# Starfish-develop/Starfish

Hardware: AMD Instinct MI355X
Metric: log-likelihood evals/sec, 4096-pixel order, batch=128 walkers (higher is better)
Workload: dtype f64; 1 GPU; cfg2: synthetic single order N_pix=4096, 8 eigenspectra, M=27, N_f=8192, 1 global + 1 local kernel, all 13 parameters thawed, batch=128 walkers per GPU; global_batch=128, units_per_gpu=128, parallelism=(order x walker) units sharded x1, one process per GPU, no data-path collective

## Files before the change

starfish_amd/csrc/sf_chol_dataflow.h:

```cpp
#pragma once
#include "sf_chol_host.h"
#include "sf_chol_diag.h"
#include "sf_chol_sync.h"
#include "sf_chol_panel.h"

struct sf_df_stage {
    int off;
    int St;
    int Sr;
    int thr_pt;
    int thr_rp;
    int dep;
    int fw;
};
struct sf_df_stage_packed {
    int off;
    unsigned short thr_pt, thr_rp, fw;
    unsigned char split;
    signed char dep;
};
static_assert(sizeof(sf_df_stage_packed) == 12, "sf_df_stage_packed");
template <class S>
__host__ __device__ __forceinline__ sf_df_stage sf_df_stage_of(S& x) {
    sf_df_stage r;
    r.off = x.off;
    const int sp = x.split;
    r.St = sp & 15;
    r.Sr = sp >> 4;
    r.thr_pt = x.thr_pt;
    r.thr_rp = x.thr_rp;
    r.dep = x.dep;
    r.fw = x.fw;
    return r;
}
static inline sf_df_stage_packed sf_df_pack(const sf_df_stage& x) {
    sf_df_stage_packed r;
    r.off = x.off;
    r.thr_pt = (unsigned short)x.thr_pt;
    r.thr_rp = (unsigned short)x.thr_rp;
    r.fw = (unsigned short)x.fw;
    r.split = (unsigned char)(x.St | (x.Sr << 4));
    r.dep = (signed char)x.dep;
    return r;
}
#define SF_DF_QUEUES 8
#define SF_DF_MAX_STAGES 127
#define SF_DF_FRONT_MAX 6
#define SF_DF_FRONT_WIDEST 3
#define SF_DF_QTILES (2 * SF_CHIP_WGS / SF_DF_QUEUES)
struct sf_df_args {
    sf_panel_args p;
    int nt, batch, front;
    int fstart[SF_DF_FRONT_MAX];
    int thr_base[2][2][SF_DF_FRONT_MAX];
    int fp_pos;
    int bq[2], ntasks[2];
    int pt_cap;
    int *head, *abort_flag, *done_top, *done_D, *done_row, *row_L, *fp_cnt, *rp_cnt, *stage_done;
    int* chain_next;
    double* T;
    int64_t sT;
    double* part;
    int* info;
    int qbal;
    long long* diag;
    long long* dbg;
    int miss_claims;
    long long* trace;
    long long trace_cap;
    sf_df_stage_packed st[2][SF_DF_MAX_STAGES];
};
static_assert(sizeof(sf_df_args) <= 4096, "kernel arguments of k_potrf_dataflow");
#define SF_DF_LDS_DOUBLES ((37 * DBS + 128) > (4 * GT * GLD + 2 * GT) ? (37 * DBS + 128) : (4 * GT * GLD + 2 * GT))
#define SF_DF_LDS_BYTES ((SF_DF_LDS_DOUBLES + 4) * sizeof(double))

typedef const __attribute__((address_space(4))) sf_df_args sf_df_kargs;
#define SF_DF_HELPER __attribute__((noinline))
#define SF_DF_PROGRESS() sf_df_add(a.abort_flag + 5, 1)
#ifdef SF_TUNING
#define SF_DF_MISS_CLAIMS(x) ((a.miss_claims & 1) && (x))
#else
#define SF_DF_MISS_CLAIMS(x) (false)
#endif
__device__ SF_DF_HELPER bool sf_df_try_chain(sf_df_kargs& a, const int qx, int& cb, int& ck, int& cd) {
    const int nt = a.nt, F = a.front;
    const int Bq = (a.batch - qx + SF_DF_QUEUES - 1) / SF_DF_QUEUES;
    const int vq = Bq == a.bq[0] ? 0 : 1;
    for (int dd = 1; dd <= F; ++dd) {
        for (int j = 0; j < Bq; ++j) {
            const int b1 = qx + SF_DF_QUEUES * j;
            int* ctr = a.chain_next + SF_DF_FRONT_MAX * b1 + dd - 1;
            const int k1 = sf_df_load(ctr);
            const int kp = dd == 1 ? k1 - 1 : k1 + a.fstart[dd - 1];
            if (dd == 1 ? k1 >= nt : kp + dd > nt - 1) continue;
            bool ready = true;
            if (kp >= 0) {
                ready = sf_df_load(a.done_top + b1) >= kp;
                if (ready && kp >= 1) {
                    ready = sf_df_load(a.row_L + (size_t)b1 * nt + kp + dd) >= kp;
                    const int St = a.st[vq][kp - 1].split & 15;
                    if (ready && St > 0)
                        ready = sf_df_load(a.fp_cnt + 2 * SF_DF_FRONT_MAX * b1 + SF_DF_FRONT_MAX * (kp & 1) + dd - 1) >=
                                a.st[vq][kp - 1].thr_pt - a.thr_base[vq][kp & 1][dd - 1];
                }
            }
            if (!ready) continue;
            int expect = k1;
            if (__hip_atomic_compare_exchange_strong(ctr, &expect, k1 + 1, __ATOMIC_RELAXED, __ATOMIC_RELAXED,
                                                     __HIP_MEMORY_SCOPE_AGENT)) {
                cb = b1;
                ck = dd == 1 ? k1 : kp;
                cd = dd;
                return true;
            }
        }
    }
    return false;
}

template <bool RHS>
__global__ __launch_bounds__(512, 4) void k_potrf_dataflow(const sf_df_args a_in) {
    extern __shared__ __attribute__((aligned(16))) double dsm[];
    double* sm = dsm;
    double(*red)[GT] = (double(*)[GT])(dsm + 4 * GT * GLD);
    int* s_ints = (int*)(dsm + SF_DF_LDS_DOUBLES);
    const size_t region = sf_split_region_tiles_dev() * (size_t)(GT * GT);
    sf_df_kargs* ap = (sf_df_kargs*)__builtin_amdgcn_kernarg_segment_ptr();
    (void)a_in;
    int qcur = (int)(blockIdx.x & (SF_DF_QUEUES - 1));
    {
        const int nb = ap->batch, big = nb % SF_DF_QUEUES;
        if (ap->qbal && big != 0) {
            if (nb < SF_DF_QUEUES && SF_DF_QUEUES % nb == 0) {
                qcur = qcur % nb;
            } else {
                const int mine = (nb - qcur + SF_DF_QUEUES - 1) / SF_DF_QUEUES;
                const int slot = (int)(blockIdx.x >> 3);
                const int keep = (int)(((long long)mine * gridDim.x + nb / 2) / nb);
                if (qcur >= big && slot >= keep) qcur = (slot - keep + qcur) % big;
            }
        }
    }
    int visited = 0;
    int kst = 0;
    if (threadIdx.x == 0) {
        s_ints[5] = 0;
        s_ints[6] = 0;
        sf_df_add(ap->abort_flag + 6, 1);
        if (blockIdx.x == 0)
            __hip_atomic_store((long long*)(ap->abort_flag + 8), (long long)ap->diag, __ATOMIC_RELAXED, __HIP_MEMORY_SCOPE_AGENT);
    }
    int pend_t = -1, resume = 0;
    for (;;) {
        int tid = threadIdx.x;
        asm volatile("" : "+v"(tid));
        sf_df_kargs& a = *ap;
        const int nt = a.nt, F = a.front;
        const int n = a.p.n, fp = a.p.fp;
        const int B = (a.batch - qcur + SF_DF_QUEUES - 1) / SF_DF_QUEUES;
        const int v = B == a.bq[0] ? 0 : 1;
        const int ntasks = B > 0 ? a.ntasks[v] : 0;
        if (resume) {
            resume = 0;
        } else if (pend_t >= 0) {
            if (tid == 0) s_ints[0] = pend_t;
            pend_t = -1;
        } else if (tid == 0) {
            int t = -1, cb = 0, ck = 0, cd = 1;
            if (sf_df_load(a.abort_flag) == 0) {
                t = -2;
                auto try_chain = [&](int qx) { return SF_DF_MISS_CLAIMS(visited < SF_DF_QUEUES) ? false : sf_df_try_chain(a, qx, cb, ck, cd); };
                if (try_chain(qcur)) {
                    t = -3;
                } else if (visited < SF_DF_QUEUES) {
                    t = ntasks > 0 ? __hip_atomic_fetch_add(a.head + qcur, 1, __ATOMIC_RELAXED, __HIP_MEMORY_SCOPE_AGENT) : ntasks;
                    if (t >= ntasks) t = -4;
                } else {
                    bool live = false;
                    for (int qx = 0; qx < SF_DF_QUEUES && t == -2; ++qx)
                        if (try_chain(qx)) {
                            t = -3;
                            s_ints[5] = 0;
                        }
                    if (t == -2) {
                        for (int b1 = 0; b1 < a.batch; ++b1) {
                            live = live || sf_df_load(a.chain_next + SF_DF_FRONT_MAX * b1) < nt;
                            for (int dd = 2; dd <= F; ++dd)
                                live = live || sf_df_load(a.chain_next + SF_DF_FRONT_MAX * b1 + dd - 1) + a.fstart[dd - 1] + dd <= nt - 1;
                        }
                        if (!live) {
                            t = -5;
                        } else {
                            const int now = (int)((wall_clock64() >> 20) & 0x3fffffff) + 1;
                            const int pg = sf_df_load(a.abort_flag + 5);
                            if (s_ints[5] == 0 || pg != s_ints[6]) {
                                s_ints[5] = now;
                                s_ints[6] = pg;
                            }
                            const int idle = (now - s_ints[5]) & 0x3fffffff;
                            const int stall = (int)(sf_df_stall_ticks(a.abort_flag) >> 20);
                            if (idle > stall) {
                                sf_df_report(a.abort_flag, a.chain_next, nt, SF_DF_ABORT_STALL, (long long)idle << 20);
                                t = -1;
                            }
                            __builtin_amdgcn_s_sleep(64);
                        }
                    }
                }
            }
            s_ints[0] = t;
            s_ints[2] = cb;
            s_ints[3] = ck;
            s_ints[4] = cd;
        }
        __syncthreads();
        const int t = __builtin_amdgcn_readfirstlane(s_ints[0]);
        const int chain_b = __builtin_amdgcn_readfirstlane(s_ints[2]), chain_k = __builtin_amdgcn_readfirstlane(s_ints[3]);
        const int chain_d = __builtin_amdgcn_readfirstlane(s_ints[4]);
        __syncthreads();
        if (t == -1) {
            if (a.info)
                for (int bb = tid; bb < a.batch; bb += 512) a.info[bb] = SF_INFO_INTERNAL;
            return;
        }
        if (t == -5) return;
        if (t == -2) continue;
// ... 617 lines not shown
```

starfish_amd/csrc/sf_chol_host.h:

```cpp
#pragma once
#include "sf_chol_tile.h"

#define SF_TSKEW 40
#define SF_CHIP_WGS 512
#define SF_SPLIT_MAX 8
static size_t sf_split_region_tiles(void) { return 2 * SF_CHIP_WGS; }
__device__ __forceinline__ size_t sf_split_region_tiles_dev(void) { return 2 * SF_CHIP_WGS; }
static int sf_split_policy(long long wgs, int nk) {
    int S = 1;
    while (2 * S <= SF_SPLIT_MAX && wgs * 2 * S <= 384 && nk / (2 * S) >= 8) S *= 2;
    return S;
}
struct sf_potrf_scratch {
    double* T;
    int64_t sT;
    double* W;
    int64_t sW;
    double* part;
    int batch;
    size_t doubles;
    double* Wbuf(int i) const { return W + (size_t)i * batch * sW; }
    size_t Wdoubles() const { return 2 * (size_t)batch * sW; }
    double* Wslot(int k) const { return Wbuf((k >> 1) & 1) + (size_t)(k & 1) * GT * SF_LDT; }
};
static sf_potrf_scratch sf_potrf_scratch_of(double* work, int n, int batch) {
    sf_potrf_scratch w = {};
    const size_t b = (size_t)batch;
    w.sT = (int64_t)(n + SF_NB) * SF_LDT + SF_TSKEW;
    w.sW = (int64_t)SF_NB * SF_LDT + SF_TSKEW;
    w.batch = batch;
    const size_t oT = b * SF_LTB_DOUBLES, oW = oT + b * w.sT, opart = oW + w.Wdoubles() + 64;
    w.doubles = opart + (size_t)(SF_EXEC_GROUPS + 1) * sf_split_region_tiles() * (GT * GT);
    if (work) {
        w.T = work + oT;
        w.W = work + oW;
        w.part = work + opart;
    }
    return w;
}
size_t sf_potrf_work_doubles(int n, int batch) { return sf_potrf_scratch_of(nullptr, n, batch).doubles; }

template <class Args>
static void sf_set_gen(Args& g, const sf_gen_args* gen, int fp) {
    if (!gen) return;
    g.genY = gen->Y - fp;
    g.sY = (int64_t)gen->mpad * gen->ldy;
    g.ldy = gen->ldy;
    g.mpad = gen->mpad;
    g.tilemap = gen->tilemap;
    g.nt128 = gen->nt128;
}
template <class Args>
static Args sf_panel_frame(double* A, int n, int lda, int64_t stride, double* rhs, int ldr, const sf_gen_args* gen, int fp) {
    Args g = {};
    g.C = A;
    g.sC = stride;
    g.lda = lda;
    g.n = n;
    g.rhs = rhs;
    g.ldr = ldr;
    g.fp = fp;
    sf_set_gen(g, gen, fp);
    return g;
}

#define SF_TRY(x)          \
    do {                   \
        int rc__ = (x);    \
        if (rc__) return rc__; \
    } while (0)
static int sf_exec_fork(sf_exec* ex, hipStream_t s, std::initializer_list<hipStream_t> to) {
    hipEvent_t e;
    SF_TRY(sf_exec_event(ex, &e));
    SF_HIP(hipEventRecord(e, s));
    for (hipStream_t t : to) SF_HIP(hipStreamWaitEvent(t, e, 0));
    return SF_OK;
}
static int sf_exec_join(sf_exec* ex, hipStream_t s, hipStream_t c, std::initializer_list<hipEvent_t> also = {}) {
    hipEvent_t e;
    SF_TRY(sf_exec_event(ex, &e));
    SF_HIP(hipEventRecord(e, c));
    SF_HIP(hipStreamWaitEvent(s, e, 0));
    for (hipEvent_t x : also)
        if (x) SF_HIP(hipStreamWaitEvent(s, x, 0));
    return SF_OK;
}
```

starfish_amd/csrc/sf_chol_panel.h:

```cpp
#pragma once
#include "sf_device.h"
#include "sf_chol_tile.h"

struct sf_panel_args {
    double* C;
    int64_t sC;
    int lda, n;
    int k0, pw;
    int row0, nslab;
    int slab_step;
    int ksplit, kchunk;
    double* part;
    const double* Wt;
    int64_t sW;
    double* rhs;
    int ldr;
    double* Sout;
    int64_t sS;
    int ldS;
    const double* genY;
    const unsigned char* tilemap;
    int64_t sY;
    int ldy, mpad, nt128;
    int kband, nband, xrow0;
    int fp;
    int prio;
    int kstop, ktail;
    const int* wflag;
    int wval;
    int* abort_flag;
};

struct sf_panel_task {
    int k0, pw, row0, nslab, slab_step;
    int ksplit, kchunk, kstop, ktail;
    double* part;
    const double* Wt;
    int64_t sW;
    double* Sout;
    const int* wflag;
    int wval;
    int* abort_flag;
    int* lds_int;
    int* top_flag;
    int top_val;
    const int* sflag;
    int sval;
    long long* stamps;
    int prio;
};
__device__ __forceinline__ sf_panel_task sf_task_of(const sf_panel_args& g) {
    sf_panel_task q;
    q.k0 = g.k0;
    q.pw = g.pw;
    q.row0 = g.row0;
    q.nslab = g.nslab;
    q.slab_step = g.slab_step;
    q.ksplit = g.ksplit;
    q.kchunk = g.kchunk;
    q.kstop = g.kstop;
    q.ktail = g.ktail;
    q.part = g.part;
    q.Wt = g.Wt;
    q.sW = g.sW;
    q.Sout = g.Sout;
    q.wflag = g.wflag;
    q.wval = g.wval;
    q.abort_flag = g.abort_flag;
    q.lds_int = nullptr;
    q.top_flag = nullptr;
    q.top_val = 0;
    q.sflag = nullptr;
    q.sval = 0;
    q.stamps = nullptr;
    q.prio = g.prio;
    return q;
}

__device__ __forceinline__ const double* sf_uniform_ptr(const double* p) {
    const unsigned long long v = (unsigned long long)p;
    const unsigned lo = __builtin_amdgcn_readfirstlane((unsigned)v), hi = __builtin_amdgcn_readfirstlane((unsigned)(v >> 32));
    return (const double*)(((unsigned long long)hi << 32) | lo);
}

__device__ __forceinline__ int sf_swz(int row) {
    const int t = (row >> 1) & 7;
    return t ^ ((((t >> 1) ^ (t >> 2)) & 1) << 1);
}

template <int NI_LO>
__device__ __forceinline__ void sf_solve_step(sf_d4 (&acc)[2][4], const double* Ab, const double* Bb) {
#pragma unroll
    for (int ks = 0; ks < 4; ++ks) {
        double a[2], bb[4];
#pragma unroll
        for (int i = 0; i < 2; ++i) a[i] = Ab[i * 16 * CLD + ks * 4];
#pragma unroll
        for (int i = NI_LO; i < 4; ++i) bb[i] = Bb[i * 16 * GLD + ks * 4];
#pragma unroll
        for (int mi = 0; mi < 2; ++mi)
#pragma unroll
            for (int ni = NI_LO; ni < 4; ++ni)
                acc[mi][ni] = __builtin_amdgcn_mfma_f64_16x16x4f64(a[mi], bb[ni], acc[mi][ni], 0, 0, 0);
    }
}

template <bool RHS, int MODE, class GA>
__device__ __forceinline__ void sf_panel_body(GA& g, const sf_panel_task& tk, const int id, double* __restrict__ sm,
                                              double (*red)[GT], const int tid) {
    constexpr int TM = 2, TN = 4;
    double(*As)[GT * GLD] = (double(*)[GT * GLD]) sm;
    double(*Bs)[GT * GLD] = (double(*)[GT * GLD])(sm + 2 * GT * GLD);
    double* Ach = sm;

    const int tile = __builtin_amdgcn_readfirstlane(MODE == 1 ? id / tk.ksplit : id);
    const int sp = __builtin_amdgcn_readfirstlane(MODE == 1 ? id - tile * tk.ksplit : 0);
    const int b = __builtin_amdgcn_readfirstlane(tile / tk.nslab);
    const int sl = tile - b * tk.nslab;
    const int row0 = (g.xrow0 && sl == tk.nslab - 1) ? g.xrow0 : tk.row0 + sl * tk.slab_step * GT;
    const int rows_here = min(GT, ((g.nband && row0 < g.nband) ? g.nband : g.n) - row0);
    const int pw = tk.pw, k0 = tk.k0;
    const int cfp = k0 == 0 ? g.fp : 0;
    if (tk.prio) __builtin_amdgcn_s_setprio(2);

    const int lane = tid & 63;
    const int w = __builtin_amdgcn_readfirstlane(tid >> 6);
    const int wm = w >> 1, wn = (w ^ (w >> 2)) & 1;
    const int l15 = lane & 15, lq = lane >> 4;
    double* Cb = g.C + (int64_t)b * g.sC;

    sf_d4 acc[TM][TN];
    if (pw > 0) {
        const int lr = tid >> 3, lc = (tid & 7) * 2;
        const double* Ap[2];
        const double* Bp[2];
#pragma unroll
        for (int p = 0; p < 2; ++p) {
            Ap[p] = Cb + (int64_t)(row0 + min(lr + 64 * p, rows_here - 1)) * g.lda + lc;
            Bp[p] = Cb + (int64_t)(k0 + min(lr + 64 * p, pw - 1)) * g.lda + lc;
        }
        const int grow = lane >> 3, gpos = lane & 7;
        unsigned Aoff[2], Boff[2];
        const double* Abase = sf_uniform_ptr(Cb + (int64_t)row0 * g.lda);
        const double* Bbase = sf_uniform_ptr(Cb + (int64_t)k0 * g.lda);
#pragma unroll
        for (int q = 0; q < 2; ++q) {
            const int row = 16 * w + 8 * q + grow;
            const int c = gpos ^ sf_swz(row);
            Aoff[q] = (unsigned)(min(row, rows_here - 1) * g.lda + 2 * c) * 8u;
            Boff[q] = (unsigned)(min(row, pw - 1) * g.lda + 2 * c) * 8u;
        }
        typedef __attribute__((address_space(3))) void* lds_ptr;
        double* A2 = sm;
        double* B2 = sm + 2 * GT * GK;
        const unsigned ldsA = (unsigned)(size_t)(lds_ptr)A2, ldsB = (unsigned)(size_t)(lds_ptr)B2;
// ... 231 lines not shown
#ifdef SF_TUNING
                if (tk.stamps) tk.stamps[2] = wall_clock64();
#endif
            }
        }
        if (RHS && g.rhs) {
            const double* z = g.rhs + (int64_t)b * g.ldr + k0;
            double zc[TN];
#pragma unroll
            for (int ni = 0; ni < TN; ++ni) {
                const int col = wn * (16 * TN) + ni * 16 + l15;
                zc[ni] = (col < pw && col >= cfp) ? z[col] : 0.0;
            }
#pragma unroll
            for (int mi = 0; mi < TM; ++mi)
#pragma unroll
                for (int r = 0; r < 4; ++r) {
                    double v = 0.0;
#pragma unroll
                    for (int ni = 0; ni < TN; ++ni) v = __builtin_fma(acc[mi][ni][r], zc[ni], v);
                    v += __shfl_xor(v, 1);
                    v += __shfl_xor(v, 2);
                    v += __shfl_xor(v, 4);
                    v += __shfl_xor(v, 8);
                    if (l15 == 0) red[wn][wm * (16 * TM) + mi * 16 + lq + 4 * r] = v;
                }
        }
    }

    {
        const int p = w >> 1, h = w & 1;
        int bi[5], bj[5];
#pragma unroll
        for (int q = 0; q < 5; ++q) {
            if (h == 0) {
                bi[q] = 7 - p;
                bj[q] = q;
            } else {
                const int n_hi = 3 - p;
                const int qq = q < 4 ? q : 0;
                bi[q] = qq < n_hi ? 7 - p : p;
                bj[q] = qq < n_hi ? 5 + qq : qq - n_hi;
            }
        }
        const int nstore = h == 0 ? 5 : 4;
        const int nk2 = pw / GK;
        const int lr = tid >> 3, lc = (tid & 7) * 2;
        const double* Lp[2];
#pragma unroll
        for (int q = 0; q < 2; ++q) Lp[q] = Cb + (int64_t)(row0 + min(lr + 64 * q, rows_here - 1)) * g.lda + k0 + lc;
        double2 rl[2];
        auto gload2 = [&](int kt) {
#pragma unroll
            for (int q = 0; q < 2; ++q) rl[q] = kt * GK + lc >= cfp ? *(const double2*)(Lp[q] + kt * GK) : make_double2(0.0, 0.0);
        };
        auto lstore2 = [&](int buf) {
#pragma unroll
            for (int q = 0; q < 2; ++q) {
                double* pa = &As[buf][(lr + 64 * q) * GLD + lc];
                pa[0] = rl[q].x;
                pa[1] = rl[q].y;
            }
        };
        if (tk.sflag && !sf_df_wait(tk.sflag, tk.sval, tk.abort_flag, tid, tk.lds_int)) return;
#ifdef SF_TUNING
        if (tk.stamps && tid == 0) tk.stamps[3] = wall_clock64();
#endif
        __syncthreads();
        if (nk2 > 0) gload2(0);
        const double* Sin = Cb + (int64_t)row0 * g.lda + row0;
        sf_d4 acc2[5];
        const bool full_tile = rows_here == GT && row0 >= g.fp;
        if (full_tile) {
#pragma unroll
            for (int q = 0; q < 5; ++q)
#pragma unroll
                for (int r = 0; r < 4; ++r) {
                    const int row = 16 * bi[q] + lq + 4 * r, col = 16 * bj[q] + l15;
                    acc2[q][r] = Sin[(int64_t)row * g.lda + col];
                }
        } else {
#pragma unroll
            for (int q = 0; q < 5; ++q)
#pragma unroll
                for (int r = 0; r < 4; ++r) {
                    const int row = 16 * bi[q] + lq + 4 * r, col = 16 * bj[q] + l15;
                    if (row0 + min(row, col) < g.fp)
                        acc2[q][r] = row == col ? 1.0 : 0.0;
                    else
                        acc2[q][r] = (q < nstore && row < rows_here && col < rows_here) ? Sin[(int64_t)row * g.lda + col] : 0.0;
                }
        }
        if (nk2 > 0) lstore2(0);
        __syncthreads();
        auto compute2 = [&](int cur) {
            const double* S = &As[cur][l15 * GLD + lq];
#pragma unroll
            for (int ks = 0; ks < GK / 4; ++ks) {
#pragma unroll
                for (int q = 0; q < 5; ++q)
                    acc2[q] = __builtin_amdgcn_mfma_f64_16x16x4f64(S[bi[q] * 16 * GLD + ks * 4], S[bj[q] * 16 * GLD + ks * 4],
                                                                   acc2[q], 0, 0, 1);
            }
        };
        for (int kt = 0; kt + 1 < nk2; ++kt) {
            gload2(kt + 1);
            compute2(kt & 1);
            lstore2((kt & 1) ^ 1);
            __syncthreads();
        }
        if (nk2 > 0) compute2((nk2 - 1) & 1);
        const bool parked = tk.Sout && sl == 0;
        double* So = parked ? tk.Sout + (int64_t)b * g.sS : Cb + (int64_t)row0 * g.lda + row0;
        const int ldo = parked ? g.ldS : g.lda;
        if (full_tile) {
#pragma unroll
            for (int q = 0; q < 4; ++q)
#pragma unroll
                for (int r = 0; r < 4; ++r) {
                    const int row = 16 * bi[q] + lq + 4 * r, col = 16 * bj[q] + l15;
                    So[(int64_t)row * ldo + col] = acc2[q][r];
                }
            if (nstore == 5) {
#pragma unroll
                for (int r = 0; r < 4; ++r) {
                    const int row = 16 * bi[4] + lq + 4 * r, col = 16 * bj[4] + l15;
                    So[(int64_t)row * ldo + col] = acc2[4][r];
                }
            }
        } else {
#pragma unroll
            for (int q = 0; q < 5; ++q) {
                if (q >= nstore) continue;
#pragma unroll
                for (int r = 0; r < 4; ++r) {
                    const int row = 16 * bi[q] + lq + 4 * r, col = 16 * bj[q] + l15;
                    if (row < rows_here && col < rows_here) So[(int64_t)row * ldo + col] = acc2[q][r];
                }
            }
        }
    }
    if (RHS && g.rhs && pw > 0) {
        __syncthreads();
        if (tid < rows_here) g.rhs[(int64_t)b * g.ldr + row0 + tid] -= red[0][tid] + red[1][tid];
    }
}

template <bool RHS, int MODE>
__global__ __launch_bounds__(512, 4) void k_chol_panel(sf_panel_args g) {
    __shared__ __attribute__((aligned(16))) double sm[4 * GT * GLD];
    __shared__ double red[2][GT];
    sf_panel_body<RHS, MODE>(g, sf_task_of(g), sf_xcd_remap(blockIdx.x, gridDim.x), sm, red, threadIdx.x);
}
```

starfish_amd/csrc/sf_chol_seq.h:

```cpp
#pragma once
#include "sf_chol_host.h"
#include "sf_chol_diag.h"
#include "sf_chol_panel.h"
#include "sf_chol_wide.h"

static int sf_check_front_pad(int fp, int n) {
    if (fp != 0 && (fp != 64 || n % GT != 64)) {
        sf_set_error("potrf: front pad %d does not fit n = %d", fp, n);
        return SF_EINVAL;
    }
    return SF_OK;
}

template <class Args>
static void sf_park(Args& g, const sf_potrf_scratch& ws) {
    g.Sout = ws.T;
    g.sS = ws.sT;
    g.ldS = SF_LDT;
}
static double sf_slab_rows(int n, int row0, int nslab, int step) {
    double rows = 0.0;
    for (int i = 0; i < nslab; ++i) {
        const int r0 = row0 + i * step * GT;
        rows += (n - r0 < GT) ? n - r0 : GT;
    }
    return rows;
}
static int sf_check_grid(long long nblk) {
    if (nblk > 0x7fffffffLL) {
        sf_set_error("panel grid too large");
        return SF_EINVAL;
    }
    return SF_OK;
}

static int sf_panel_split(int k0, int pw, int fp, long long nblk) {
    return pw > 0 ? sf_split_policy(nblk, (k0 > fp ? k0 - fp : 0) / GK) : 1;
}
static int sf_panel_step(sf_panel_args g, const sf_potrf_scratch& ws, int k0, int pw, int row0, int nslab, int step, const double* Wt,
                         bool to_scratch, hipStream_t st, int region, int phase) {
    const int n = g.n, fp = g.fp, batch = ws.batch;
    g.k0 = k0;
    g.pw = pw;
    g.row0 = row0;
    g.nslab = nslab;
    g.slab_step = step;
    g.Wt = Wt;
    g.sW = ws.sW;
    if (to_scratch) {
        sf_park(g, ws);
        g.prio = 1;
    }
    const long long nblk = (long long)nslab * batch;
    SF_TRY(sf_check_grid(nblk));
    const double rows = sf_slab_rows(n, row0, nslab, step);
    const double flops_main = 2.0 * (k0 > fp ? k0 - fp : 0) * rows * pw * batch;
    const double flops_epi = (rows * pw * (double)pw + (double)GT * rows * pw) * batch;
    const int nk = (k0 > fp ? k0 - fp : 0) / GK;
    const int S = sf_panel_split(k0, pw, fp, nblk);
    void* tok;
    if (S > 1) {
        g.ksplit = S;
        g.kchunk = (nk + S - 1) / S;
        g.part = ws.part + (size_t)region * sf_split_region_tiles() * (GT * GT);
        if (phase != 2) {
            sf_prof_gemm_begin(st, flops_main, &tok);
            hipLaunchKernelGGL((k_chol_panel<false, 1>), dim3((unsigned)(nblk * S)), dim3(512), 0, st, g);
            sf_prof_gemm_end(tok);
        }
        if (phase != 1) {
            sf_prof_gemm_begin(st, flops_epi, &tok);
            if (g.rhs)
                hipLaunchKernelGGL((k_chol_panel<true, 2>), dim3((unsigned)nblk), dim3(512), 0, st, g);
            else
                hipLaunchKernelGGL((k_chol_panel<false, 2>), dim3((unsigned)nblk), dim3(512), 0, st, g);
            sf_prof_gemm_end(tok);
        }
    } else {
        sf_prof_gemm_begin(st, flops_main + flops_epi, &tok);
        if (g.rhs)
            hipLaunchKernelGGL((k_chol_panel<true, 0>), dim3((unsigned)nblk), dim3(512), 0, st, g);
        else
            hipLaunchKernelGGL((k_chol_panel<false, 0>), dim3((unsigned)nblk), dim3(512), 0, st, g);
        sf_prof_gemm_end(tok);
    }
    SF_LAUNCH_CHECK();
    return SF_OK;
}

struct sf_wide_stamps {
#ifdef SF_TUNING
    long long* t = nullptr;
    int n = 0, k[64];
#endif
};
#ifdef SF_TUNING
static int sf_wide_stamps_begin(sf_wide_stamps& w) {
    if (SF_TUNE_FLAG("SF_WIDE_STAMPS")) {
        SF_HIP(hipHostMalloc((void**)&w.t, sizeof(long long) * 16 * 64));
        for (int i = 0; i < 16 * 64; ++i) w.t[i] = 0;
    }
    return SF_OK;
}
static void sf_wide_stamps_report(sf_wide_stamps& w, hipStream_t s) {
    if (!w.t) return;
    (void)hipStreamSynchronize(s);
    fprintf(stderr, "wide launches, workgroup grid/2: k nslab | prologue | K loop | solve 1 | 2b | solve 2 | store + rhs | S load + step 4 | S store + drain | total (us)\n");
    for (int i = 0; i < w.n; ++i) {
        const long long* t = w.t + 16 * i;
        fprintf(stderr, "%2d %2d |", w.k[i] / 1000, w.k[i] % 1000);
        const int seg[8][2] = {{0, 1}, {1, 2}, {2, 3}, {3, 4}, {4, 5}, {5, 6}, {6, 7}, {7, 8}};
        for (auto& sg : seg) fprintf(stderr, " %7.1f |", (t[sg[1]] - t[sg[0]]) / 100.0);
        fprintf(stderr, " %7.1f\n", (t[8] - t[0]) / 100.0);
    }
    (void)hipHostFree(w.t);
}
#else
static int sf_wide_stamps_begin(sf_wide_stamps&) { return SF_OK; }
static void sf_wide_stamps_report(sf_wide_stamps&, hipStream_t) {}
#endif

static int sf_panel_step_w(sf_panelw_args g, const sf_potrf_scratch& ws, int k, int slab0, int nslab, int step, bool park, hipStream_t st,
                           sf_wide_stamps& stamps) {
    const int n = g.n, fp = g.fp, batch = ws.batch;
    g.k0 = k * GT;
    g.row0 = slab0 * GT;
    g.nslab = nslab;
    g.slab_step = step;
    g.Wt0 = ws.Wslot(k);
    g.Wt1 = ws.Wslot(k + 1);
    g.sW = ws.sW;
    if (park) sf_park(g, ws);
    const long long nblk = (long long)nslab * batch;
    SF_TRY(sf_check_grid(nblk));
#ifdef SF_TUNING
    if (stamps.t && stamps.n < 64) {
        stamps.k[stamps.n] = k * 1000 + nslab;
        g.stamps = stamps.t + 16 * stamps.n++;
    }
#endif
    const double rows = sf_slab_rows(n, g.row0, nslab, step);
    const double kk = g.k0 > fp ? g.k0 - fp : 0;
    const double flops = (2.0 * kk * rows * GT + 2.0 * (kk + GT) * rows * GT + 2.0 * (rows * GT * (double)GT + (double)GT * rows * GT)) * batch;
    void* tok;
    sf_prof_gemm_begin(st, flops, &tok);
    if (g.rhs)
        hipLaunchKernelGGL(k_chol_panel_w<true>, dim3((unsigned)nblk), dim3(1024), SF_PANELW_LDS, st, g);
    else
        hipLaunchKernelGGL(k_chol_panel_w<false>, dim3((unsigned)nblk), dim3(1024), SF_PANELW_LDS, st, g);
    sf_prof_gemm_end(tok);
    SF_LAUNCH_CHECK();
    return SF_OK;
}

static int sf_diag_step(const sf_potrf_scratch& ws, double* A, int lda, int64_t stride, double* rhs, int ldr, int* info, int n, int k,
                        double* Wt, int fp, hipStream_t st) {
    const int k0 = k * GT;
    const int pw = (n - k0 < GT) ? n - k0 : GT;
    return sf_launch_diag128(ws.T, ws.sT, pw, info, k0 - fp, rhs ? rhs + k0 : nullptr, ldr, A + (int64_t)k0 * lda + k0, lda, stride, Wt,
                             ws.sW, ws.batch, st, k == 0 ? fp : 0);
}

struct sf_narrow_events {
    hipEvent_t d, rest[2];
};
static int sf_narrow_step(const sf_panel_args& base, const sf_potrf_scratch& ws, sf_exec* ex, int* info, int k, double* Wt, hipStream_t c,
                          const hipStream_t gs[2], const hipEvent_t last[2], hipEvent_t* e_top, sf_narrow_events* ev) {
    const int n = base.n, fp = base.fp, nt = (n + GT - 1) / GT;
    const int k0 = k * GT;
    const int pw = (n - k0 < GT) ? n - k0 : GT;
    *ev = {};
    SF_TRY(sf_diag_step(ws, base.C, base.lda, base.sC, base.rhs, base.ldr, info, n, k, Wt, fp, c));
    if (k + 1 >= nt) return SF_OK;
    SF_TRY(sf_exec_event(ex, &ev->d));
    SF_HIP(hipEventRecord(ev->d, c));
    const int gk = (k + 1) & 1;
    if (e_top && sf_panel_split(k0, pw, fp, ws.batch) > 1) {
        if (*e_top) SF_HIP(hipStreamWaitEvent(gs[gk], *e_top, 0));
        SF_TRY(sf_panel_step(base, ws, k0, pw, (k + 1) * GT, 1, 1, Wt, true, gs[gk], 0, 1));
        hipEvent_t e_part;
        SF_TRY(sf_exec_event(ex, &e_part));
        SF_HIP(hipEventRecord(e_part, gs[gk]));
        SF_HIP(hipStreamWaitEvent(c, e_part, 0));
        SF_TRY(sf_panel_step(base, ws, k0, pw, (k + 1) * GT, 1, 1, Wt, true, c, 0, 2));
    } else {
        if (last[gk]) SF_HIP(hipStreamWaitEvent(c, last[gk], 0));
        SF_TRY(sf_panel_step(base, ws, k0, pw, (k + 1) * GT, 1, 1, Wt, true, c, 0, 0));
    }
    if (e_top) {
        SF_TRY(sf_exec_event(ex, e_top));
        SF_HIP(hipEventRecord(*e_top, c));
    }
    for (int g = 0; g < 2; ++g) {
        const int first = k + 2 + (((k + 2) & 1) != g);
        if (first >= nt) continue;
        const int cnt = (nt - 1 - first) / 2 + 1;
        SF_HIP(hipStreamWaitEvent(gs[g], ev->d, 0));
        SF_TRY(sf_panel_step(base, ws, k0, pw, first * GT, cnt, 2, Wt, false, gs[g], 1 + g, 0));
        SF_TRY(sf_exec_event(ex, &ev->rest[g]));
        SF_HIP(hipEventRecord(ev->rest[g], gs[g]));
    }
    return SF_OK;
}

static int sf_launch_potrf_v2(double* A, int n, int lda, int64_t stride, int* info, const sf_potrf_scratch& ws, double* rhs,
                              int ldr, hipStream_t s, const sf_gen_args* gen, sf_exec* ex, int fp) {
    const int batch = ws.batch;
    SF_HIP(hipMemsetAsync(info, 0, sizeof(int) * (size_t)batch, s));
    SF_TRY(sf_exec_prepare(ex));
    constexpr int G = 2;
    hipStream_t c = ex->side;
    const hipStream_t gs[G] = {s, ex->grp[0]};
    SF_TRY(sf_exec_fork(ex, s, {c, gs[1]}));

    const sf_panel_args base = sf_panel_frame<sf_panel_args>(A, n, lda, stride, rhs, ldr, gen, fp);
    const int nt = (n + GT - 1) / GT;
    SF_TRY(sf_panel_step(base, ws, 0, 0, 0, 1, 1, nullptr, true, c, 0, 0));
    hipEvent_t e_epi = nullptr;
    hipEvent_t e_rest[G] = {};
    hipEvent_t e_rest_prev[G] = {};
    for (int k = 0; k < nt; ++k) {
        for (int g = 0; g < G; ++g)
            if (e_rest_prev[g]) SF_HIP(hipStreamWaitEvent(c, e_rest_prev[g], 0));
        sf_narrow_events ev;
        SF_TRY(sf_narrow_step(base, ws, ex, info, k, ws.Wbuf(k & 1), c, gs, e_rest, &e_epi, &ev));
        for (int g = 0; g < G; ++g) {
            e_rest_prev[g] = e_rest[g];
            if (ev.rest[g]) e_rest[g] = ev.rest[g];
        }
    }
    SF_TRY(sf_exec_join(ex, s, c, {e_rest[1]}));
    return SF_OK;
}

static int sf_launch_potrf_v3(double* A, int n, int lda, int64_t stride, int* info, const sf_potrf_scratch& ws, double* rhs,
                              int ldr, hipStream_t s, const sf_gen_args* gen, sf_exec* ex, bool half, int fp) {
    const int batch = ws.batch;
    static sf_dev_once attr_once;
    SF_CHECK(sf_lds_limit_once(&attr_once, 160 * 1024, {(const void*)k_chol_panel_w<true>, (const void*)k_chol_panel_w<false>}));
    SF_HIP(hipMemsetAsync(info, 0, sizeof(int) * (size_t)batch, s));
    SF_TRY(sf_exec_prepare(ex));
    hipStream_t c = ex->side, xa = ex->side;
    SF_TRY(sf_exec_fork(ex, s, {c, xa, ex->grp[0]}));
    const int nt = (n + GT - 1) / GT;

    const sf_panel_args base = sf_panel_frame<sf_panel_args>(A, n, lda, stride, rhs, ldr, gen, fp);
    const sf_panelw_args wbase = sf_panel_frame<sf_panelw_args>(A, n, lda, stride, rhs, ldr, gen, fp);
    sf_wide_stamps stamps;
    SF_TRY(sf_wide_stamps_begin(stamps));
    auto diag = [&](int k) -> int { return sf_diag_step(ws, A, lda, stride, rhs, ldr, info, n, k, ws.Wslot(k), fp, c); };

    SF_TRY(sf_panel_step(base, ws, 0, 0, 0, 1, 1, nullptr, true, c, 0, 0));
    const hipStream_t bs[2] = {s, ex->grp[0]};
    hipEvent_t e_A = nullptr;
    hipEvent_t e_last[2] = {nullptr, nullptr};
    std::vector<hipEvent_t> readers[4];
    auto wait_readers = [&](int slot) -> int {
        for (hipEvent_t e : readers[slot]) SF_HIP(hipStreamWaitEvent(c, e, 0));
        readers[slot].clear();
        return SF_OK;
    };
    int k = 0;
    for (; k < nt; k += 2) {
        if (k + 2 >= nt) break;
        if (half && k >= (nt / 4) * 2 && k > 0) break;
        if (e_A) SF_HIP(hipStreamWaitEvent(c, e_A, 0));
        SF_TRY(wait_readers(k & 3));
        SF_TRY(diag(k));
        SF_TRY(sf_panel_step(base, ws, k * GT, GT, (k + 1) * GT, 1, 1, ws.Wslot(k), true, c, 0, 0));
        SF_TRY(wait_readers((k + 1) & 3));
        SF_TRY(diag(k + 1));
        hipEvent_t e_chain;
        SF_TRY(sf_exec_event(ex, &e_chain));
        SF_HIP(hipEventRecord(e_chain, c));
        const int na = (nt - (k + 2) < 2) ? nt - (k + 2) : 2;
        SF_HIP(hipStreamWaitEvent(xa, e_chain, 0));
        for (int g = 0; g < 2; ++g)
            if (e_last[g]) SF_HIP(hipStreamWaitEvent(xa, e_last[g], 0));
        SF_TRY(sf_panel_step_w(wbase, ws, k, k + 2, na, 1, true, xa, stamps));
        SF_TRY(sf_exec_event(ex, &e_A));
        SF_HIP(hipEventRecord(e_A, xa));
        readers[k & 3].push_back(e_A);
        readers[(k + 1) & 3].push_back(e_A);
        for (int g = 0; g < 2; ++g) {
            const int first = k + 4 + g;
            if (first >= nt) continue;
            const int cnt = (nt - 1 - first) / 2 + 1;
            SF_HIP(hipStreamWaitEvent(bs[g], e_chain, 0));
            SF_TRY(sf_panel_step_w(wbase, ws, k, first, cnt, 2, false, bs[g], stamps));
            SF_TRY(sf_exec_event(ex, &e_last[g]));
            SF_HIP(hipEventRecord(e_last[g], bs[g]));
            readers[k & 3].push_back(e_last[g]);
            readers[(k + 1) & 3].push_back(e_last[g]);
        }
    }
    for (; k < nt; ++k) {
        if (e_A) {
            SF_HIP(hipStreamWaitEvent(c, e_A, 0));
            for (int g = 0; g < 2; ++g) SF_HIP(hipStreamWaitEvent(bs[g], e_A, 0));
            e_A = nullptr;
        }
        SF_TRY(wait_readers(k & 3));
        sf_narrow_events ev;
        SF_TRY(sf_narrow_step(base, ws, ex, info, k, ws.Wslot(k), c, bs, e_last, nullptr, &ev));
        for (int g = 0; g < 2; ++g)
            if (ev.rest[g]) {
                e_last[g] = ev.rest[g];
                readers[k & 3].push_back(ev.rest[g]);
            }
    }
    SF_TRY(sf_exec_join(ex, s, c, {e_A, e_last[1]}));
    sf_wide_stamps_report(stamps, s);
    return SF_OK;
}
```

starfish_amd/csrc/sf_chol_sync.h:

```cpp
#pragma once
#include "sf_common.h"

#define SF_DF_TIMEOUT_TICKS 400000000LL
#define SF_DF_STALL_TICKS 2500000LL
#define SF_DF_ABORT_TIMEOUT 1
#define SF_DF_ABORT_STALL 2
__device__ __forceinline__ int sf_df_load(const int* flag) {
    return __hip_atomic_load(flag, __ATOMIC_RELAXED, __HIP_MEMORY_SCOPE_AGENT);
}
__device__ __forceinline__ void sf_df_report(int* abort_flag, const int* f, int target, int reason = SF_DF_ABORT_TIMEOUT,
                                             long long waited = 0) {
    if (__hip_atomic_exchange(abort_flag, 1, __ATOMIC_RELAXED, __HIP_MEMORY_SCOPE_AGENT) == 0) {
        if (f) {
            abort_flag[1] = (int)(f - abort_flag);
            abort_flag[2] = target;
            abort_flag[3] = __hip_atomic_load(f, __ATOMIC_RELAXED, __HIP_MEMORY_SCOPE_AGENT);
        }
        long long* diag = (long long*)__hip_atomic_load((long long*)(abort_flag + 8), __ATOMIC_RELAXED, __HIP_MEMORY_SCOPE_AGENT);
        if (diag) {
            diag[1] = reason;
            diag[2] = sf_df_load(abort_flag + 6);
            diag[3] = gridDim.x;
            diag[4] = waited;
            diag[5] = sf_df_load(abort_flag + 5);
            __hip_atomic_fetch_add(diag, 1LL, __ATOMIC_RELEASE, __HIP_MEMORY_SCOPE_SYSTEM);
        }
    }
}
__device__ __forceinline__ long long sf_df_stall_ticks(const int* abort_flag) {
    const int o = abort_flag[7];
    return o ? (long long)o << 16 : SF_DF_STALL_TICKS;
}
#define SF_DF_RESCUE_TICKS 50000LL
#define SF_DF_DEFERRED 4
struct sf_df_no_rescue {
    __device__ __forceinline__ bool operator()() const { return false; }
};
struct sf_df_watch {
    long long t0, tp;
    int pg0;
};
__device__ __attribute__((noinline)) int sf_df_wait_slow(sf_df_watch& w, int* abort_flag, const int* f1, int t1, const int* f2, int t2,
                                                         const int* f3, int t3, const bool look_at_progress) {
    if (sf_df_load(abort_flag) != 0) return 1;
    const long long now = wall_clock64();
    const long long waited = now - w.t0;
    int reason = 0;
    if (look_at_progress) {
        const int pg = sf_df_load(abort_flag + 5);
        if (pg != w.pg0) {
            w.pg0 = pg;
            w.tp = now;
        } else if (now - w.tp > sf_df_stall_ticks(abort_flag)) {
            reason = SF_DF_ABORT_STALL;
        }
    }
    if (!reason && waited > SF_DF_TIMEOUT_TICKS && (abort_flag[4] == 0 || (waited >> 20) > abort_flag[4])) reason = SF_DF_ABORT_TIMEOUT;
    if (reason) {
        const bool m1 = f1 && sf_df_load(f1) < t1, m2 = f2 && sf_df_load(f2) < t2;
        sf_df_report(abort_flag, m1 ? f1 : (m2 ? f2 : f3), m1 ? t1 : (m2 ? t2 : t3), reason, waited);
        return 1;
    }
    return waited > SF_DF_RESCUE_TICKS ? 2 : 0;
}
template <class RESCUE>
__device__ __forceinline__ int sf_df_wait_r(const int* f1, int t1, const int* f2, int t2, const int* f3, int t3,
                                            const int* probe, int tprobe, bool* probe_ok, int* abort_flag, const int tid,
                                            int* s_okp, RESCUE&& rescue, const bool can_rescue) {
    if (tid == 0) {
        int ok = 1;
        auto ready = [&]() {
            return (!f1 || sf_df_load(f1) >= t1) && (!f2 || sf_df_load(f2) >= t2) && (!f3 || sf_df_load(f3) >= t3);
        };
        if (!ready()) {
            sf_df_watch w;
            w.t0 = w.tp = wall_clock64();
            w.pg0 = sf_df_load(abort_flag + 5);
            unsigned it = 0;
            for (;;) {
                __builtin_amdgcn_s_sleep(4);
                if (ready()) break;
                if ((++it & 31) == 0) {
                    const int r = sf_df_wait_slow(w, abort_flag, f1, t1, f2, t2, f3, t3, (it & 255) == 0);
                    if (r == 1) {
                        ok = 0;
                        break;
                    }
                    if (r == 2 && can_rescue && rescue()) {
                        ok = SF_DF_DEFERRED;
                        break;
                    }
                }
            }
        }
        if (probe && sf_df_load(probe) >= tprobe) ok |= 2;
        __builtin_amdgcn_fence(__ATOMIC_ACQUIRE, "agent");
        *s_okp = ok;
    }
    __syncthreads();
    const int ok = __builtin_amdgcn_readfirstlane(*s_okp);
    __syncthreads();
    if (probe_ok) *probe_ok = (ok & 2) != 0;
    return ok & (1 | SF_DF_DEFERRED);
}
__device__ __forceinline__ bool sf_df_wait(const int* f1, int t1, const int* f2, int t2, const int* f3, int t3,
                                           const int* probe, int tprobe, bool* probe_ok, int* abort_flag, const int tid,
                                           int* s_okp) {
    return sf_df_wait_r(f1, t1, f2, t2, f3, t3, probe, tprobe, probe_ok, abort_flag, tid, s_okp, sf_df_no_rescue(), false) == 1;
}
__device__ __forceinline__ bool sf_df_wait(const int* flag, int target, int* abort_flag, const int tid, int* s_okp) {
    return sf_df_wait(flag, target, nullptr, 0, nullptr, 0, nullptr, 0, nullptr, abort_flag, tid, s_okp);
}
__device__ __forceinline__ void sf_df_release() {
    __builtin_amdgcn_fence(__ATOMIC_RELEASE, "agent");
    asm volatile("s_waitcnt vmcnt(0)" ::: "memory");
}
__device__ __forceinline__ void sf_df_set(int* flag, int value) {
    __hip_atomic_store(flag, value, __ATOMIC_RELAXED, __HIP_MEMORY_SCOPE_AGENT);
}
__device__ __forceinline__ void sf_df_add(int* flag, int value) {
    __hip_atomic_fetch_add(flag, value, __ATOMIC_RELAXED, __HIP_MEMORY_SCOPE_AGENT);
}
```

Measured before the change: 2778 evals/s.

## Fuse diag, panel, and next diag into one chained kernel per step

Result: no change. 2779 evals/s (median of 6 runs) (+0.1%).

```diff
diff --git a/starfish_amd/csrc/sf_chol_dataflow.h b/starfish_amd/csrc/sf_chol_dataflow.h
--- a/starfish_amd/csrc/sf_chol_dataflow.h
+++ b/starfish_amd/csrc/sf_chol_dataflow.h
@@ -71,7 +71,7 @@
     sf_df_stage_packed st[2][SF_DF_MAX_STAGES];
 };
 static_assert(sizeof(sf_df_args) <= 4096, "kernel arguments of k_potrf_dataflow");
-#define SF_DF_LDS_DOUBLES ((37 * DBS + 128) > (4 * GT * GLD + 2 * GT) ? (37 * DBS + 128) : (4 * GT * GLD + 2 * GT))
+#define SF_DF_LDS_DOUBLES SF_PANEL_DIAG_LDS_DOUBLES
 #define SF_DF_LDS_BYTES ((SF_DF_LDS_DOUBLES + 4) * sizeof(double))
 
 typedef const __attribute__((address_space(4))) sf_df_args sf_df_kargs;
diff --git a/starfish_amd/csrc/sf_chol_host.h b/starfish_amd/csrc/sf_chol_host.h
--- a/starfish_amd/csrc/sf_chol_host.h
+++ b/starfish_amd/csrc/sf_chol_host.h
@@ -4,11 +4,12 @@
 #define SF_TSKEW 40
 #define SF_CHIP_WGS 512
 #define SF_SPLIT_MAX 8
+#define SF_SPLIT_WGS 384
 static size_t sf_split_region_tiles(void) { return 2 * SF_CHIP_WGS; }
 __device__ __forceinline__ size_t sf_split_region_tiles_dev(void) { return 2 * SF_CHIP_WGS; }
 static int sf_split_policy(long long wgs, int nk) {
     int S = 1;
-    while (2 * S <= SF_SPLIT_MAX && wgs * 2 * S <= 384 && nk / (2 * S) >= 8) S *= 2;
+    while (2 * S <= SF_SPLIT_MAX && wgs * 2 * S <= SF_SPLIT_WGS && nk / (2 * S) >= 8) S *= 2;
     return S;
 }
 struct sf_potrf_scratch {
diff --git a/starfish_amd/csrc/sf_chol_panel.h b/starfish_amd/csrc/sf_chol_panel.h
--- a/starfish_amd/csrc/sf_chol_panel.h
+++ b/starfish_amd/csrc/sf_chol_panel.h
@@ -1,6 +1,8 @@
 #pragma once
 #include "sf_device.h"
 #include "sf_chol_tile.h"
+#include "sf_chol_diag.h"
+#include "sf_chol_sync.h"
 
 struct sf_panel_args {
     double* C;
@@ -538,3 +540,25 @@
     __shared__ double red[2][GT];
     sf_panel_body<RHS, MODE>(g, sf_task_of(g), sf_xcd_remap(blockIdx.x, gridDim.x), sm, red, threadIdx.x);
 }
+
+#define SF_PANEL_DIAG_LDS_DOUBLES ((37 * DBS + 128) > (4 * GT * GLD + 2 * GT) ? (37 * DBS + 128) : (4 * GT * GLD + 2 * GT))
+
+template <bool RHS>
+__global__ __launch_bounds__(512, 4) void k_chol_panel_chain(sf_panel_args g, int* __restrict__ info, double* __restrict__ Wt1) {
+    extern __shared__ __attribute__((aligned(16))) double dsm[];
+    double(*red)[GT] = (double(*)[GT])(dsm + 4 * GT * GLD);
+    const int b = sf_xcd_remap(blockIdx.x, gridDim.x);
+    int tid = threadIdx.x;
+    __builtin_amdgcn_s_setprio(2);
+    auto diag = [&](int k0, double* Wt) {
+        sf_diag_lds_body(g.Sout, g.sS, GT, info, k0 - g.fp, g.rhs ? g.rhs + k0 : nullptr, g.ldr, g.C + (int64_t)k0 * g.lda + k0, g.lda,
+                         g.sC, Wt, g.sW, k0 == 0 ? g.fp : 0, b, dsm, tid);
+    };
+    diag(g.k0, const_cast<double*>(g.Wt));
+    sf_wg_reread(tid);
+    asm volatile("" : "+v"(tid));
+    sf_panel_body<RHS, 3>(g, sf_task_of(g), b, dsm, red, tid);
+    sf_wg_reread(tid);
+    asm volatile("" : "+v"(tid));
+    diag(g.k0 + GT, Wt1);
+}
diff --git a/starfish_amd/csrc/sf_chol_seq.h b/starfish_amd/csrc/sf_chol_seq.h
--- a/starfish_amd/csrc/sf_chol_seq.h
+++ b/starfish_amd/csrc/sf_chol_seq.h
@@ -159,6 +159,44 @@
     const int pw = (n - k0 < GT) ? n - k0 : GT;
     return sf_launch_diag128(ws.T, ws.sT, pw, info, k0 - fp, rhs ? rhs + k0 : nullptr, ldr, A + (int64_t)k0 * lda + k0, lda, stride, Wt,
                              ws.sW, ws.batch, st, k == 0 ? fp : 0);
+}
+
+static int sf_chain_step(sf_panel_args g, const sf_potrf_scratch& ws, int* info, int k, hipStream_t st) {
+    static sf_dev_once attr_once;
+    SF_CHECK(sf_lds_limit_once(&attr_once, 160 * 1024, {(const void*)k_chol_panel_chain<true>, (const void*)k_chol_panel_chain<false>}));
+    const int batch = ws.batch;
+    SF_TRY(sf_check_grid(batch));
+    g.k0 = k * GT;
+    g.pw = GT;
+    g.row0 = (k + 1) * GT;
+    g.nslab = 1;
+    g.slab_step = 1;
+    g.Wt = ws.Wslot(k);
+    g.sW = ws.sW;
+    sf_park(g, ws);
+    g.prio = 1;
+    const int nk = (g.k0 > g.fp ? g.k0 - g.fp : 0) / GK;
+    const int S = sf_panel_split(g.k0, GT, g.fp, batch);
+    const double flops_main = 2.0 * nk * GK * GT * GT * batch, flops_epi = 2.0 * GT * GT * (double)GT * batch;
+    void* tok;
+    if (S > 1) {
+        g.ksplit = S;
+        g.kchunk = (nk + S - 1) / S;
+        g.part = ws.part;
+        g.ktail = g.k0 / GK;
+        sf_prof_gemm_begin(st, flops_main, &tok);
+        hipLaunchKernelGGL((k_chol_panel<false, 1>), dim3((unsigned)(batch * S)), dim3(512), 0, st, g);
+        sf_prof_gemm_end(tok);
+    }
+    const size_t lds = SF_PANEL_DIAG_LDS_DOUBLES * sizeof(double);
+    sf_prof_gemm_begin(st, (S > 1 ? 0.0 : flops_main) + flops_epi, &tok);
+    if (g.rhs)
+        hipLaunchKernelGGL(k_chol_panel_chain<true>, dim3((unsigned)batch), dim3(512), lds, st, g, info, ws.Wslot(k + 1));
+    else
+        hipLaunchKernelGGL(k_chol_panel_chain<false>, dim3((unsigned)batch), dim3(512), lds, st, g, info, ws.Wslot(k + 1));
+    sf_prof_gemm_end(tok);
+    SF_LAUNCH_CHECK();
+    return SF_OK;
 }
 
 struct sf_narrow_events {
@@ -248,8 +286,6 @@
     const sf_panelw_args wbase = sf_panel_frame<sf_panelw_args>(A, n, lda, stride, rhs, ldr, gen, fp);
     sf_wide_stamps stamps;
     SF_TRY(sf_wide_stamps_begin(stamps));
-    auto diag = [&](int k) -> int { return sf_diag_step(ws, A, lda, stride, rhs, ldr, info, n, k, ws.Wslot(k), fp, c); };
-
     SF_TRY(sf_panel_step(base, ws, 0, 0, 0, 1, 1, nullptr, true, c, 0, 0));
     const hipStream_t bs[2] = {s, ex->grp[0]};
     hipEvent_t e_A = nullptr;
@@ -266,10 +302,8 @@
         if (half && k >= (nt / 4) * 2 && k > 0) break;
         if (e_A) SF_HIP(hipStreamWaitEvent(c, e_A, 0));
         SF_TRY(wait_readers(k & 3));
-        SF_TRY(diag(k));
-        SF_TRY(sf_panel_step(base, ws, k * GT, GT, (k + 1) * GT, 1, 1, ws.Wslot(k), true, c, 0, 0));
         SF_TRY(wait_readers((k + 1) & 3));
-        SF_TRY(diag(k + 1));
+        SF_TRY(sf_chain_step(base, ws, info, k, c));
         hipEvent_t e_chain;
         SF_TRY(sf_exec_event(ex, &e_chain));
         SF_HIP(hipEventRecord(e_chain, c));
diff --git a/starfish_amd/csrc/sf_chol_sync.h b/starfish_amd/csrc/sf_chol_sync.h
--- a/starfish_amd/csrc/sf_chol_sync.h
+++ b/starfish_amd/csrc/sf_chol_sync.h
@@ -115,6 +115,16 @@
     __builtin_amdgcn_fence(__ATOMIC_RELEASE, "agent");
     asm volatile("s_waitcnt vmcnt(0)" ::: "memory");
 }
+__device__ __forceinline__ void sf_wg_reread(const int tid) {
+    asm volatile("s_waitcnt vmcnt(0)" ::: "memory");
+    __syncthreads();
+    if (tid == 0) {
+        sf_df_release();
+        __builtin_amdgcn_fence(__ATOMIC_ACQUIRE, "agent");
+        asm volatile("s_waitcnt vmcnt(0)" ::: "memory");
+    }
+    __syncthreads();
+}
 __device__ __forceinline__ void sf_df_set(int* flag, int value) {
     __hip_atomic_store(flag, value, __ATOMIC_RELAXED, __HIP_MEMORY_SCOPE_AGENT);
 }
```
